# eladhoffer/convNet.pytorch

Hardware: NVIDIA H100
Metric: ResNet-50 images/sec (training step, synthetic 224x224) (higher is better)
Workload: dtype bf16

## Files before the change

convnet/pytorch_b200/csrc/conv3x3.cu:

```cuda
#include "common.cuh"
#include "host.h"
#include <stdlib.h>

namespace b200 {

constexpr int kHThreads = 384;
constexpr int kHTileM = 128;
constexpr int kHMaxA = 6, kHMaxB = 8;
constexpr int kHMaxTaps = 16;
constexpr int kHStatReplicas = 16;

struct HaloParams {
  int N, H, W, C, Kout;
  int RT, Wp;
  int tiles_per_img, m_tiles, n_tiles, block_n, c_chunks;
  int sa, sb;
  uint32_t a_bytes, a_box_bytes, b_bytes;
  int act;
  int has_res;
  double* stats;
  const float* bias;
  int ntaps, pad;
  int row_bytes;
  int b_stationary;
  int diag;
  uint16_t a_off[kHMaxTaps];
  uint16_t b_tap[kHMaxTaps];
};

template <int NTAPS, int KSTEPS, int BN>
__global__ void __launch_bounds__(kHThreads, 1)
conv_halo_kernel(const __grid_constant__ CUtensorMap tmX, const __grid_constant__ CUtensorMap tmB,
                 const __grid_constant__ CUtensorMap tmC, const __grid_constant__ CUtensorMap tmR,
                 const __grid_constant__ HaloParams p) {
  extern __shared__ uint8_t smem_raw[];
  __shared__ __align__(8) uint64_t a_full[kHMaxA], a_empty[kHMaxA], b_full[kHMaxB], b_empty[kHMaxB];
  __shared__ __align__(8) uint64_t res_bar, bstat_bar;

  const int warp = threadIdx.x >> 5, lane = threadIdx.x & 31;
  const uint32_t raw_addr = smem_u32(smem_raw);
  uint8_t* smem = smem_raw + (((raw_addr + 1023u) & ~1023u) - raw_addr);
  uint8_t* sA = smem;
  uint8_t* sB = sA + p.sa * p.a_bytes;
  const int b_slots = p.b_stationary ? p.c_chunks * p.ntaps : p.sb;
  uint8_t* epi = sB + b_slots * p.b_bytes;

  if (threadIdx.x == 0) {
    for (int i = 0; i < p.sa; ++i) { mbar_init(&a_full[i], 1); mbar_init(&a_empty[i], 8); }
    for (int i = 0; i < kHMaxB; ++i) { mbar_init(&b_full[i], 1); mbar_init(&b_empty[i], 8); }
    mbar_init(&bstat_bar, 1);
    mbar_init(&res_bar, 1);
    fence_mbar_init();
    prefetch_tmap(&tmX); prefetch_tmap(&tmB); prefetch_tmap(&tmC);
    if (p.has_res) prefetch_tmap(&tmR);
  }
  __syncthreads();
  const int t_start = p.diag ? static_cast<int>(blockIdx.x) / p.n_tiles : static_cast<int>(blockIdx.x);
  const int t_step = p.diag ? static_cast<int>(gridDim.x) / p.n_tiles : static_cast<int>(gridDim.x);
  const int total_tiles = p.diag ? p.m_tiles : p.m_tiles * p.n_tiles;
  const int own_n = static_cast<int>(blockIdx.x) % p.n_tiles;

  if (warp >= 8) {
    producer_setmaxnreg();
    if (warp == 8 && lane == 0) {
      int ia = 0, ib = 0; uint32_t pa = 0, pb = 0;
      const int cw = p.row_bytes >> 1;
      if (p.b_stationary && t_start < total_tiles) {
        mbar_arrive_expect_tx(&bstat_bar, static_cast<uint32_t>(p.c_chunks * NTAPS) * p.b_bytes);
        for (int cc = 0; cc < p.c_chunks; ++cc)
          for (int t = 0; t < NTAPS; ++t)
            tma_load_3d(&tmB, &bstat_bar, sB + (cc * NTAPS + t) * p.b_bytes, cc * cw, p.b_tap[t],
                        p.diag ? own_n * p.block_n : 0);
      }
      for (int tile = t_start; tile < total_tiles; tile += t_step) {
        const int m_tile = p.diag ? tile : tile / p.n_tiles, n_tile = p.diag ? own_n : tile - m_tile * p.n_tiles;
        const int img = m_tile / p.tiles_per_img;
        const int h0 = (m_tile - img * p.tiles_per_img) * p.RT;
        for (int cc = 0; cc < p.c_chunks; ++cc) {
          mbar_wait(&a_empty[ia], pa ^ 1u);
          mbar_arrive_expect_tx(&a_full[ia], p.a_box_bytes);
          tma_load_4d(&tmX, &a_full[ia], sA + ia * p.a_bytes, (p.diag ? n_tile : cc) * cw, -p.pad, h0 - p.pad, img);
          if (++ia == p.sa) { ia = 0; pa ^= 1u; }
          if (p.b_stationary) continue;
          for (int t = 0; t < NTAPS; ++t) {
            mbar_wait(&b_empty[ib], pb ^ 1u);
            mbar_arrive_expect_tx(&b_full[ib], p.b_bytes);
            tma_load_3d(&tmB, &b_full[ib], sB + ib * p.b_bytes, cc * cw, p.b_tap[t], n_tile * p.block_n);
            if (++ib == p.sb) { ib = 0; pb ^= 1u; }
          }
        }
      }
    }
    return;
  }
  consumer_setmaxnreg();

  const int wg = warp >> 2;
  const int r_lo = wg * 64 + (warp & 3) * 16 + (lane >> 2);
  const int c_lo = 2 * (lane & 3);
  const bool leader = threadIdx.x == 0;
  const uint64_t proto = make_smem_desc(0, 16, 8u * p.row_bytes, layout_type_for_row_bytes(p.row_bytes));
  const uint32_t a_wg = (64u * wg * p.row_bytes) >> 4;
  const int nbox = BN >> 6;
  const uint32_t box_bytes = static_cast<uint32_t>(p.RT * p.W) * 128u;
  const uint32_t box_pitch = (box_bytes + 1023u) & ~1023u;
  int srow[2];
  bool in_tile[2];
#pragma unroll
  for (int h = 0; h < 2; ++h) {
    const int v = r_lo + 8 * h;
    const int ry = v / p.Wp, cx = v - ry * p.Wp;
    srow[h] = ry * p.W + cx;
    in_tile[h] = (ry < p.RT) && (cx < p.W);
  }
  const int st_col = threadIdx.x % BN;
  const int st_rows = kHTileM / (256 / BN);
  const int st_row0 = (threadIdx.x / BN) * st_rows;
  int st_ntile = -1;
  float st_s1 = 0.f, st_s2 = 0.f;
  if (p.b_stationary && t_start < total_tiles) mbar_wait(&bstat_bar, 0);

  float acc[BN / 2];
  int ia = 0, ib = 0; uint32_t pa = 0, pb = 0;
  int local = 0;
  for (int tile = t_start; tile < total_tiles; tile += t_step, ++local) {
    const int m_tile = p.diag ? tile : tile / p.n_tiles, n_tile = p.diag ? own_n : tile - m_tile * p.n_tiles;
    const int img = m_tile / p.tiles_per_img;
    const int h0 = (m_tile - img * p.tiles_per_img) * p.RT;
    const int nbase = n_tile * BN;
    if (leader && local > 0) bulk_wait_group_read0();
    named_bar_sync(1, 256);
    if (leader && p.has_res) {
      fence_proxy_async();
      mbar_arrive_expect_tx(&res_bar, static_cast<uint32_t>(nbox) * box_bytes);
      for (int b = 0; b < nbox; ++b) tma_load_4d(&tmR, &res_bar, epi + b * box_pitch, nbase + b * 64, 0, h0, img);
    }

    wgmma_fence_acc(acc);
    int rel_a = -1, rel_b = -1;
    for (int cc = 0; cc < p.c_chunks; ++cc) {
      mbar_wait(&a_full[ia], pa);
      const uint64_t da0 = proto + (smem_u32(sA + ia * p.a_bytes) >> 4) + a_wg;
#pragma unroll
      for (int t = 0; t < NTAPS; ++t) {
        uint64_t db0;
        if (p.b_stationary) {
          db0 = proto + (smem_u32(sB + (cc * NTAPS + t) * p.b_bytes) >> 4);
        } else {
          mbar_wait(&b_full[ib], pb);
          db0 = proto + (smem_u32(sB + ib * p.b_bytes) >> 4);
        }
        const uint32_t tap_inc = (static_cast<uint32_t>(p.a_off[t]) * p.row_bytes) >> 4;
        wgmma_fence();
#pragma unroll
        for (int k = 0; k < KSTEPS; ++k)
          wgmma_bf16<0, 0>(acc, da0 + tap_inc + 2 * k, db0 + 2 * k, (cc | t | k) != 0 ? 1u : 0u);
        if (!p.b_stationary || t == NTAPS - 1) {
          wgmma_commit();
          wgmma_wait<1>();
          if (rel_b >= 0) release_stage(&b_empty[rel_b], lane);
          if (rel_a >= 0) release_stage(&a_empty[rel_a], lane);
          rel_a = (t == NTAPS - 1) ? ia : -1;
          rel_b = p.b_stationary ? -1 : ib;
        }
        if (!p.b_stationary && ++ib == p.sb) { ib = 0; pb ^= 1u; }
      }
      if (++ia == p.sa) { ia = 0; pa ^= 1u; }
    }
    wgmma_wait<0>();
    wgmma_fence_acc(acc);
    if (rel_b >= 0) release_stage(&b_empty[rel_b], lane);
    if (rel_a >= 0) release_stage(&a_empty[rel_a], lane);

    if (p.has_res) mbar_wait(&res_bar, static_cast<uint32_t>(local & 1));
#pragma unroll
    for (int h = 0; h < 2; ++h) {
      if (!in_tile[h] || h0 + (r_lo + 8 * h) / p.Wp >= p.H) continue;
      const int row = srow[h];
#pragma unroll
      for (int j = 0; j < BN / 2; j += 4) {
        const int c = 2 * j + c_lo;
        {
          uint32_t* dst = reinterpret_cast<uint32_t*>(epi + (c >> 6) * box_pitch + row * 128 +
                                                      ((((c & 63) >> 3) ^ (row & 7)) << 4) + (c & 7) * 2);
          float v0 = acc[j + 2 * h], v1 = acc[j + 2 * h + 1];
          if (p.bias != nullptr) { v0 += __ldg(p.bias + nbase + c); v1 += __ldg(p.bias + nbase + c + 1); }
          if (p.has_res) {
            const float2 t2 = unpack_bf16x2(*dst);
            v0 += t2.x;
            v1 += t2.y;
          }
          *dst = pack_bf16x2(apply_act(v0, p.act), apply_act(v1, p.act));
        }
      }
    }
    fence_proxy_async();
    named_bar_sync(1, 256);
    if (leader) {
      for (int b = 0; b < nbox; ++b) tma_store_4d(&tmC, epi + b * box_pitch, nbase + b * 64, 0, h0, img);
      bulk_commit_group();
    }
    if (p.stats != nullptr) {
      if (st_ntile != n_tile) {
        if (st_ntile >= 0) {
          double* dst = p.stats + (blockIdx.x % kHStatReplicas) * 2 * p.Kout + st_ntile * BN + st_col;
          atomicAdd(dst, (double)st_s1);
          atomicAdd(dst + p.Kout, (double)st_s2);
        }
        st_ntile = n_tile; st_s1 = 0.f; st_s2 = 0.f;
      }
      const int vrows = min(p.RT, p.H - h0) * p.W;
      const uint8_t* col = epi + (st_col >> 6) * box_pitch + (st_col & 7) * 2;
      const int j = (st_col & 63) >> 3;
      const int r_end = min(st_row0 + st_rows, vrows);
      for (int r = st_row0; r < r_end; ++r) {
        const float x = __bfloat162float(*reinterpret_cast<const __nv_bfloat16*>(col + r * 128 + ((j ^ (r & 7)) << 4)));
        st_s1 += x;
        st_s2 = fmaf(x, x, st_s2);
      }
    }
  }
  if (p.stats != nullptr && st_ntile >= 0) {
    double* dst = p.stats + (blockIdx.x % kHStatReplicas) * 2 * p.Kout + st_ntile * BN + st_col;
    atomicAdd(dst, (double)st_s1);
    atomicAdd(dst + p.Kout, (double)st_s2);
  }
  if (leader) bulk_wait_group0();
}

typedef void (*HaloKernelFn)(const __grid_constant__ CUtensorMap, const __grid_constant__ CUtensorMap,
                             const __grid_constant__ CUtensorMap, const __grid_constant__ CUtensorMap,
                             const __grid_constant__ HaloParams);
static HaloKernelFn halo_kernel_for(int ntaps, int block_n) {
  if (ntaps == 9)
    return block_n == 64 ? conv_halo_kernel<9, 4, 64> : block_n == 128 ? conv_halo_kernel<9, 4, 128>
         : block_n == 256 ? conv_halo_kernel<9, 4, 256> : nullptr;
  if (ntaps == 16)
    return block_n == 64 ? conv_halo_kernel<16, 1, 64> : block_n == 128 ? conv_halo_kernel<16, 1, 128>
         : block_n == 256 ? conv_halo_kernel<16, 1, 256> : nullptr;
  return nullptr;
}

static int enc4(CUtensorMap* tm, const void* base, int C, int W, int H, int N, int b0, int b1, int b2) {
  EncodeTiledFn fn = encode_tiled_fn();
  B200_REQUIRE(fn != nullptr, B200_ERR_CUDA, "cuTensorMapEncodeTiled entry point unavailable");
  cuuint64_t dims[4] = {(cuuint64_t)C, (cuuint64_t)W, (cuuint64_t)H, (cuuint64_t)N};
  cuuint64_t strides[3] = {(cuuint64_t)C * 2, (cuuint64_t)W * C * 2, (cuuint64_t)H * W * C * 2};
  cuuint32_t box[4] = {(cuuint32_t)b0, (cuuint32_t)b1, (cuuint32_t)b2, 1};
  cuuint32_t es[4] = {1, 1, 1, 1};
  CUresult r = fn(tm, CU_TENSOR_MAP_DATA_TYPE_BFLOAT16, 4, const_cast<void*>(base), dims, strides, box, es,
                  CU_TENSOR_MAP_INTERLEAVE_NONE, swizzle_for_row_bytes(b0 * 2), CU_TENSOR_MAP_L2_PROMOTION_L2_128B,
                  CU_TENSOR_MAP_FLOAT_OOB_FILL_NONE);
  B200_REQUIRE(r == CUDA_SUCCESS, B200_ERR_CUDA, "cuTensorMapEncodeTiled(4d) failed (%d) dims=(%d,%d,%d,%d) box=(%d,%d,%d)",
               (int)r, C, W, H, N, b0, b1, b2);
  return B200_OK;
}

bool halo_geometry_ok(int H, int W, int Cs, int R, int S, int pad) {
  const bool k3 = (R == 3 && S == 3 && pad == 1 && Cs % 64 == 0);
  const bool k4 = (R == 4 && S == 4 && pad == 0 && Cs == 16);
  if (!k3 && !k4) return false;
  const int Wp = W + S - 1;
  if (Wp > 128 || W < 8) return false;
  int RT = 128 / Wp;
  if (RT > H) RT = H;
  const int tiles = (H + RT - 1) / RT;
  return (double)H * W / (128.0 * tiles) >= 0.6;
}

bool halo_eligible(int H, int W, int Cs, int Nout, int R, int S, int pad) {
  if (!halo_geometry_ok(H, W, Cs, R, S, pad) || Nout % 64 != 0) return false;
  const int n_tiles = (Nout + 255) / 256;
  const int block_n = Nout / n_tiles;
  return Nout % n_tiles == 0 && block_n % 64 == 0 && 256 % block_n == 0;
}

int launch_halo(const void* src, const void* wmat, void* out, const void* res, const float* bias, int N, int H, int W,
                int Cs, int Nout, int R, int S, int pad, int dir, int act, double* stats, cudaStream_t stream, int window) {
  HaloParams p;
  memset(&p, 0, sizeof(p));
  p.diag = window > 0 ? 1 : 0;
  if (p.diag)
    B200_REQUIRE(window == 64 && Cs == Nout && Cs % 64 == 0 && R == 3 && S == 3, B200_ERR_UNSUPPORTED,
                 "conv halo: window mode needs window == 64, C == K, C %% 64 == 0 and a 3x3 filter (C=%d K=%d)", Cs, Nout);
  p.N = N; p.H = H; p.W = W; p.C = Cs; p.Kout = Nout;
  p.ntaps = R * S; p.pad = pad;
  p.row_bytes = (Cs == 16) ? 32 : 128;
  const int cw = p.row_bytes / 2;
  p.Wp = W + S - 1;
  p.RT = 128 / p.Wp;
  if (p.RT > H) p.RT = H;
  p.tiles_per_img = (H + p.RT - 1) / p.RT;
  p.m_tiles = N * p.tiles_per_img;
  p.n_tiles = p.diag ? Nout / 64 : (Nout + 255) / 256;
  p.block_n = Nout / p.n_tiles;
  p.c_chunks = p.diag ? 1 : Cs / cw;
  p.a_box_bytes = (uint32_t)(p.RT + R - 1) * p.Wp * p.row_bytes;
  uint32_t a_need = (uint32_t)(kHTileM + (R - 1) * p.Wp + (S - 1)) * p.row_bytes;
  if (a_need < p.a_box_bytes) a_need = p.a_box_bytes;
  p.a_bytes = (a_need + 1023u) & ~1023u;
  p.b_bytes = (uint32_t)p.block_n * p.row_bytes;
  p.act = act;
  p.has_res = res != nullptr;
  p.stats = stats;
  p.bias = bias;
  for (int r = 0; r < R; ++r)
    for (int s = 0; s < S; ++s) {
      const int t = r * S + s;
      p.b_tap[t] = (uint16_t)t;
      p.a_off[t] = (uint16_t)(dir == 0 ? r * p.Wp + s : (R - 1 - r) * p.Wp + (S - 1 - s));
    }
  const uint32_t box_pitch = (((uint32_t)(p.RT * W) * 128u) + 1023u) & ~1023u;
  const uint32_t epi_bytes = (uint32_t)(p.block_n / 64) * box_pitch;
  int budget = 212 * 1024 - (int)epi_bytes;
  const int b_all = p.c_chunks * p.ntaps * (int)p.b_bytes;
  p.b_stationary = ((p.n_tiles == 1 || p.diag) && b_all <= 80 * 1024) ? 1 : 0;
  B200_REQUIRE(!p.diag || p.b_stationary, B200_ERR_UNSUPPORTED, "conv halo: window mode expects resident weights");
  int b_region;
  if (p.b_stationary) {
    b_region = b_all;
    p.sb = 0;
    p.sa = (budget - b_region) / (int)p.a_bytes;
    if (p.sa > kHMaxA) p.sa = kHMaxA;
  } else {
    p.sa = 2;
    p.sb = (budget - p.sa * (int)p.a_bytes) / (int)p.b_bytes;
    if (p.sb > kHMaxB) p.sb = kHMaxB;
    if (p.sb >= 6 && (int)(3 * p.a_bytes + 4 * p.b_bytes) <= budget) {
      p.sa = 3;
      p.sb = (budget - 3 * (int)p.a_bytes) / (int)p.b_bytes;
      if (p.sb > kHMaxB) p.sb = kHMaxB;
    }
    b_region = p.sb * (int)p.b_bytes;
  }
  B200_REQUIRE(p.sa >= 2 && (p.b_stationary || p.sb >= 2), B200_ERR_UNSUPPORTED,
               "conv halo: shared memory budget exceeded (W=%d, block_n=%d)", W, p.block_n);
  CUtensorMap tmX, tmB, tmC, tmR;
  memset(&tmR, 0, sizeof(tmR));
  int rc = enc4(&tmX, src, Cs, W + S - 1 - 2 * pad, H + R - 1 - 2 * pad, N, cw, p.Wp, p.RT + R - 1);
  if (rc) return rc;
  {
    EncodeTiledFn fn = encode_tiled_fn();
    const int wc = p.diag ? window : Cs;
    cuuint64_t dims[3] = {(cuuint64_t)wc, (cuuint64_t)p.ntaps, (cuuint64_t)Nout};
    cuuint64_t strides[2] = {(cuuint64_t)wc * 2, (cuuint64_t)wc * p.ntaps * 2};
    cuuint32_t box[3] = {(cuuint32_t)cw, 1, (cuuint32_t)p.block_n};
    cuuint32_t es[3] = {1, 1, 1};
    CUresult r = fn(&tmB, CU_TENSOR_MAP_DATA_TYPE_BFLOAT16, 3, const_cast<void*>(wmat), dims, strides, box, es,
                    CU_TENSOR_MAP_INTERLEAVE_NONE, swizzle_for_row_bytes(p.row_bytes),
                    CU_TENSOR_MAP_L2_PROMOTION_L2_128B, CU_TENSOR_MAP_FLOAT_OOB_FILL_NONE);
    B200_REQUIRE(r == CUDA_SUCCESS, B200_ERR_CUDA, "conv halo: weight tensor map failed (%d)", (int)r);
  }
  rc = enc4(&tmC, out, Nout, W, H, N, 64, W, p.RT);
  if (rc) return rc;
  if (res) {
    rc = enc4(&tmR, res, Nout, W, H, N, 64, W, p.RT);
    if (rc) return rc;
  }
  const int smem_bytes = p.sa * (int)p.a_bytes + b_region + (int)epi_bytes + 1024;
  HaloKernelFn kfn = halo_kernel_for(p.ntaps, p.block_n);
  B200_REQUIRE(kfn != nullptr, B200_ERR_UNSUPPORTED, "conv halo: %d taps with block_n %d unsupported", p.ntaps, p.block_n);
  cudaError_t e = cudaFuncSetAttribute((const void*)kfn, cudaFuncAttributeMaxDynamicSharedMemorySize, smem_bytes);
  B200_REQUIRE(e == cudaSuccess, B200_ERR_CUDA, "conv halo: smem attribute (%d bytes): %s", smem_bytes, cudaGetErrorString(e));
  const int total = p.m_tiles * p.n_tiles;
  int grid = total < sm_count() ? total : sm_count();
  if (p.diag) {
    int per_n = sm_count() / p.n_tiles;
    if (per_n > p.m_tiles) per_n = p.m_tiles;
    if (per_n < 1) per_n = 1;
    grid = per_n * p.n_tiles;
  }
  if (getenv("B200_HALO_DEBUG"))
    fprintf(stderr, "[halo] dir=%d N=%d H=%d W=%d C=%d K=%d taps=%d block_n=%d n_tiles=%d m_tiles=%d bstat=%d diag=%d "
            "sa=%d sb=%d bias=%d res=%d act=%d stats=%d grid=%d\n", dir, N, H, W, Cs, Nout, p.ntaps, p.block_n,
            p.n_tiles, p.m_tiles, p.b_stationary, p.diag, p.sa, p.sb, bias != nullptr, res != nullptr, act,
            stats != nullptr, grid);
  b200::launch(kfn, grid, kHThreads, smem_bytes, stream, tmX, tmB, tmC, tmR, p);
  B200_CHECK_LAUNCH("conv_halo_kernel");
  return B200_OK;
}


constexpr int kWThreads = 384;
constexpr int kWMaxStages = 4;

struct HaloWgradParams {
  int N, H, W, K_out, C;
  int RT, Wp, tiles_per_img, m_tiles;
  int ntaps, pad, halo_rows;
  int x_row_bytes, cw, ncols;
  int c_chunks, k_tiles, units, splits, tiles_per_split;
  int stages;
  int window;
  uint32_t a_box_bytes, a_bytes, x_box_bytes, x_bytes;
  float* partial;
  uint16_t x_off[kHMaxTaps];
};

template <int R, int S>
__global__ void __launch_bounds__(kWThreads, 1)
conv_halo_wgrad_kernel(const __grid_constant__ CUtensorMap tmDy, const __grid_constant__ CUtensorMap tmX,
                       const __grid_constant__ HaloWgradParams p) {
  constexpr int kCols = S * 16;
  extern __shared__ uint8_t smem_raw[];
  __shared__ __align__(8) uint64_t full_bar[kWMaxStages], empty_bar[kWMaxStages];
  const int warp = threadIdx.x >> 5, lane = threadIdx.x & 31;
  const uint32_t raw_addr = smem_u32(smem_raw);
  uint8_t* smem = smem_raw + (((raw_addr + 1023u) & ~1023u) - raw_addr);
  const uint32_t stage_bytes = p.a_bytes + p.x_bytes;

  {
    uint4* z = reinterpret_cast<uint4*>(smem);
    const int n16 = static_cast<int>(p.stages * stage_bytes) >> 4;
    for (int i = threadIdx.x; i < n16; i += kWThreads) z[i] = make_uint4(0u, 0u, 0u, 0u);
  }
  if (threadIdx.x == 0) {
    for (int s = 0; s < p.stages; ++s) { mbar_init(&full_bar[s], 1); mbar_init(&empty_bar[s], 8); }
    fence_mbar_init();
    prefetch_tmap(&tmDy);
    prefetch_tmap(&tmX);
  }
  fence_proxy_async();
  __syncthreads();

  const int split = blockIdx.x / p.units;
  const int unit = blockIdx.x - split * p.units;
  const int k_tile = unit % p.k_tiles;
  const int cc = unit / p.k_tiles;
  const int k0 = k_tile * kHTileM;
  const int t_begin = split * p.tiles_per_split;
  const int t_end = min(p.m_tiles, t_begin + p.tiles_per_split);
  const int ntiles = t_end - t_begin;
  const int nA = min(2, (p.K_out - k0 + 63) / 64);
  if (ntiles <= 0) return;

  if (warp >= 8) {
    producer_setmaxnreg();
    if (warp == 8 && lane == 0) {
      int stage = 0; uint32_t phase = 0;
      const uint32_t tx = nA * p.a_box_bytes + p.x_box_bytes;
      for (int tile = t_begin; tile < t_end; ++tile) {
        const int img = tile / p.tiles_per_img;
        const int h0 = (tile - img * p.tiles_per_img) * p.RT;
        mbar_wait(&empty_bar[stage], phase ^ 1u);
        uint8_t* sa = smem + stage * stage_bytes;
        mbar_arrive_expect_tx(&full_bar[stage], tx);
        for (int j = 0; j < nA; ++j) tma_load_4d(&tmDy, &full_bar[stage], sa + j * 16384, k0 + j * 64, 0, h0, img);
        tma_load_4d(&tmX, &full_bar[stage], sa + p.a_bytes, cc * p.cw + (p.window ? k0 : 0), -p.pad, h0 - p.pad, img);
        if (++stage == p.stages) { stage = 0; phase ^= 1u; }
      }
    }
    return;
  }
  consumer_setmaxnreg();

  const int wg = warp >> 2;
  const bool wg_on = wg < nA;
  const uint64_t protoA = make_smem_desc(0, 16384, 1024, 1);
  const uint64_t protoX = make_smem_desc(0, p.x_row_bytes, 8u * p.x_row_bytes, layout_type_for_row_bytes(p.x_row_bytes));
  uint32_t row_inc[R];
#pragma unroll
  for (int r = 0; r < R; ++r) row_inc[r] = (static_cast<uint32_t>(p.x_off[r * S]) * p.x_row_bytes) >> 4;
  const uint32_t kx_inc = (16u * p.x_row_bytes) >> 4;
  float acc[R][kCols / 2];
#pragma unroll
  for (int r = 0; r < R; ++r) wgmma_fence_acc(acc[r]);
  int stage = 0, prev = 0; uint32_t phase = 0;
  for (int i = 0; i < ntiles; ++i) {
    mbar_wait(&full_bar[stage], phase);
    if (wg_on) {
      const uint32_t a_addr = smem_u32(smem + stage * stage_bytes);
      const uint64_t da0 = protoA + ((a_addr + wg * 16384) >> 4);
      const uint64_t dx0 = protoX + ((a_addr + p.a_bytes) >> 4);
      wgmma_fence();
#pragma unroll
      for (int k = 0; k < 8; ++k) {
        const uint32_t scale = (k != 0 || i != 0) ? 1u : 0u;
#pragma unroll
        for (int r = 0; r < R; ++r)
          wgmma_bf16<1, 1>(acc[r], da0 + k * 128, dx0 + row_inc[r] + k * kx_inc, scale);
      }
      wgmma_commit();
      wgmma_wait<1>();
    }
    if (i > 0) release_stage(&empty_bar[prev], lane);
    prev = stage;
    if (++stage == p.stages) { stage = 0; phase ^= 1u; }
  }
  wgmma_wait<0>();
#pragma unroll
  for (int r = 0; r < R; ++r) wgmma_fence_acc(acc[r]);
  release_stage(&empty_bar[prev], lane);
  if (!wg_on) return;

  const int row = wg * 64 + (warp & 3) * 16 + (lane >> 2);
  const int c_lo = 2 * (lane & 3);
#pragma unroll
  for (int h = 0; h < 2; ++h) {
    float* dst = p.partial + ((static_cast<long long>(unit) * p.splits + split) * kHTileM + row + 8 * h) * p.ncols;
#pragma unroll
    for (int r = 0; r < R; ++r)
#pragma unroll
      for (int j = 0; j < kCols / 2; j += 4)
        *reinterpret_cast<float2*>(dst + r * kCols + 2 * j + c_lo) = make_float2(acc[r][j + 2 * h], acc[r][j + 2 * h + 1]);
  }
}

__global__ void __launch_bounds__(256) conv_halo_wgrad_reduce_kernel(const float* __restrict__ partial,
                                                                     float* __restrict__ dw, int K_out, int ntaps, int C,
                                                                     int cw, int k_tiles, int splits, int ncols) {
  __shared__ float4 red[8][32];
  const int c4n = C >> 2;
  const long long total = static_cast<long long>(K_out) * ntaps * c4n;
  const int lane = threadIdx.x & 31, w = threadIdx.x >> 5, nw = blockDim.x >> 5;
  for (long long base = static_cast<long long>(blockIdx.x) * 32; base < total; base += static_cast<long long>(gridDim.x) * 32) {
    const long long idx = base + lane;
    float4 acc = make_float4(0.f, 0.f, 0.f, 0.f);
    int c = 0, tap = 0, k = 0;
    if (idx < total) {
      c = static_cast<int>(idx % c4n) * 4;
      tap = static_cast<int>((idx / c4n) % ntaps);
      k = static_cast<int>(idx / (static_cast<long long>(c4n) * ntaps));
      const int k_tile = k >> 7, row = k & 127;
      const int cc = c / cw;
      const int unit = cc * k_tiles + k_tile;
      const float* src = partial + ((static_cast<long long>(unit) * splits) * kHTileM + row) * ncols + tap * cw + (c - cc * cw);
      for (int s2 = w; s2 < splits; s2 += nw) {
        const float4 v = __ldcg(reinterpret_cast<const float4*>(src + static_cast<long long>(s2) * kHTileM * ncols));
        acc.x += v.x; acc.y += v.y; acc.z += v.z; acc.w += v.w;
      }
    }
    red[w][lane] = acc;
    __syncthreads();
    if (w == 0 && idx < total) {
      for (int j = 1; j < nw; ++j) {
        const float4 v = red[j][lane];
        acc.x += v.x; acc.y += v.y; acc.z += v.z; acc.w += v.w;
      }
      float4* d = reinterpret_cast<float4*>(dw + (static_cast<long long>(k) * ntaps + tap) * C + c);
      float4 o = *d;
      o.x += acc.x; o.y += acc.y; o.z += acc.z; o.w += acc.w;
      *d = o;
    }
    __syncthreads();
  }
}

bool halo_wgrad_eligible(int H, int W, int C, int K_out, int R, int S, int pad) {
  if (!halo_geometry_ok(H, W, C, R, S, pad)) return false;
  return K_out % 64 == 0;
}

int launch_halo_wgrad(const void* x, const void* dy, float* dw, void* workspace, size_t workspace_bytes, int N, int H,
                      int W, int C, int K_out, int R, int S, int pad, cudaStream_t stream, int window) {
  HaloWgradParams p;
  memset(&p, 0, sizeof(p));
  p.window = window;
  if (window)
    B200_REQUIRE(window == 128 && C == K_out && C % 128 == 0, B200_ERR_UNSUPPORTED,
                 "conv halo wgrad: window mode needs window == 128 and C == K, C %% 128 == 0 (C=%d K=%d)", C, K_out);
  p.N = N; p.H = H; p.W = W; p.K_out = K_out; p.C = C;
  p.ntaps = R * S; p.pad = pad;
  p.cw = 16;
  p.x_row_bytes = p.cw * 2;
  p.ncols = p.ntaps * p.cw;
  p.Wp = W + S - 1;
  p.RT = 128 / p.Wp;
  if (p.RT > H) p.RT = H;
  p.halo_rows = p.RT + R - 1;
  p.tiles_per_img = (H + p.RT - 1) / p.RT;
  p.m_tiles = N * p.tiles_per_img;
  p.c_chunks = (window ? window : C) / p.cw;
  p.k_tiles = (K_out + kHTileM - 1) / kHTileM;
  p.units = p.c_chunks * p.k_tiles;
  int splits = sm_count() / p.units;
  if (splits < 1) splits = 1;
  if (splits > p.m_tiles) splits = p.m_tiles;
  p.tiles_per_split = (p.m_tiles + splits - 1) / splits;
  p.splits = (p.m_tiles + p.tiles_per_split - 1) / p.tiles_per_split;
  p.a_box_bytes = (uint32_t)(p.RT * p.Wp) * 128u;
  p.a_bytes = 2 * 16384;
  p.x_box_bytes = (uint32_t)(p.halo_rows * p.Wp) * p.x_row_bytes;
  int max_off = 0;
  for (int r = 0; r < R; ++r)
    for (int s = 0; s < S; ++s) {
      p.x_off[r * S + s] = (uint16_t)(r * p.Wp + s);
      if (r * p.Wp + s > max_off) max_off = r * p.Wp + s;
    }
  uint32_t x_need = (uint32_t)(kHTileM + max_off) * p.x_row_bytes;
  if (x_need < p.x_box_bytes) x_need = p.x_box_bytes;
  p.x_bytes = (x_need + 1023u) & ~1023u;
  p.stages = (212 * 1024) / (int)(p.a_bytes + p.x_bytes);
  if (p.stages > kWMaxStages) p.stages = kWMaxStages;
  B200_REQUIRE(p.stages >= 2, B200_ERR_UNSUPPORTED, "conv halo wgrad: shared memory budget exceeded (W=%d)", W);
  const size_t need = (size_t)p.units * p.splits * kHTileM * p.ncols * sizeof(float);
  B200_REQUIRE(workspace != nullptr && workspace_bytes >= need, B200_ERR_INVALID,
               "conv halo wgrad: workspace of %zu bytes needed (%zu given)", need, workspace_bytes);
  p.partial = reinterpret_cast<float*>(workspace);
  CUtensorMap tmDy, tmX;
  int rc = enc4(&tmDy, dy, K_out, W, H, N, 64, p.Wp, p.RT);
  if (rc) return rc;
  rc = enc4(&tmX, x, C, W + S - 1 - 2 * pad, H + R - 1 - 2 * pad, N, p.cw, p.Wp, p.halo_rows);
  if (rc) return rc;
  const int smem_bytes = p.stages * (int)(p.a_bytes + p.x_bytes) + 1024;
  const void* kfn = (p.ntaps == 9) ? (const void*)conv_halo_wgrad_kernel<3, 3> : (const void*)conv_halo_wgrad_kernel<4, 4>;
  cudaError_t e = cudaFuncSetAttribute(kfn, cudaFuncAttributeMaxDynamicSharedMemorySize, smem_bytes);
  B200_REQUIRE(e == cudaSuccess, B200_ERR_CUDA, "conv halo wgrad: smem attribute (%d bytes): %s", smem_bytes,
               cudaGetErrorString(e));
  if (getenv("B200_HALO_DEBUG"))
    fprintf(stderr, "[halo_wgrad] N=%d H=%d W=%d C=%d K=%d taps=%d k_tiles=%d c_chunks=%d m_tiles=%d units=%d "
            "splits=%d tiles_per_split=%d stages=%d grid=%d\n", N, H, W, C, K_out, p.ntaps, p.k_tiles, p.c_chunks,
            p.m_tiles, p.units, p.splits, p.tiles_per_split, p.stages, p.units * p.splits);
  if (p.ntaps == 9)
    b200::launch(conv_halo_wgrad_kernel<3, 3>, p.units * p.splits, kWThreads, smem_bytes, stream, tmDy, tmX, p);
  else
    b200::launch(conv_halo_wgrad_kernel<4, 4>, p.units * p.splits, kWThreads, smem_bytes, stream, tmDy, tmX, p);
  B200_CHECK_LAUNCH("conv_halo_wgrad_kernel");
  const int Cw = window ? window : C;
  const long long total = (long long)K_out * p.ntaps * (Cw / 4);
  long long blocks64 = (total + 31) / 32;
  if (blocks64 > 16LL * sm_count()) blocks64 = 16LL * sm_count();
  const int blocks = (int)blocks64;
  b200::launch(conv_halo_wgrad_reduce_kernel, blocks, 32 * wgrad_reduce_warps(p.splits), 0, stream, p.partial, dw, K_out, p.ntaps, Cw, p.cw, p.k_tiles, p.splits,
                                                            p.ncols);
  B200_CHECK_LAUNCH("conv_halo_wgrad_reduce_kernel");
  return B200_OK;
}

}
```

Measured before the change: 6694.

## Double M tile height for block_n=64 halo conv to improve B reuse

Adds an MH template parameter so each consumer warpgroup issues two stacked 64-row wgmma per k-step, giving a 256-row M tile when block_n is 64. The host picks MH=2 if it gives more image rows per tile and still fits shared memory, and otherwise falls back to MH=1. The aim is to reuse each weight tile across twice as many output rows and cut per-tile overheads. The cost is doubled accumulator registers, a larger A buffer that may leave fewer pipeline stages, and fewer tiles, which can hurt SM load balance.

Result: faster. 6801 (median of 6 runs) (+1.6%).

```diff
diff --git a/convnet/pytorch_b200/csrc/conv3x3.cu b/convnet/pytorch_b200/csrc/conv3x3.cu
--- a/convnet/pytorch_b200/csrc/conv3x3.cu
+++ b/convnet/pytorch_b200/csrc/conv3x3.cu
@@ -28,7 +28,7 @@
   uint16_t b_tap[kHMaxTaps];
 };
 
-template <int NTAPS, int KSTEPS, int BN>
+template <int NTAPS, int KSTEPS, int BN, int MH>
 __global__ void __launch_bounds__(kHThreads, 1)
 conv_halo_kernel(const __grid_constant__ CUtensorMap tmX, const __grid_constant__ CUtensorMap tmB,
                  const __grid_constant__ CUtensorMap tmC, const __grid_constant__ CUtensorMap tmR,
@@ -96,31 +96,33 @@
   consumer_setmaxnreg();
 
   const int wg = warp >> 2;
-  const int r_lo = wg * 64 + (warp & 3) * 16 + (lane >> 2);
+  const int r_lo = wg * 64 * MH + (warp & 3) * 16 + (lane >> 2);
   const int c_lo = 2 * (lane & 3);
   const bool leader = threadIdx.x == 0;
   const uint64_t proto = make_smem_desc(0, 16, 8u * p.row_bytes, layout_type_for_row_bytes(p.row_bytes));
-  const uint32_t a_wg = (64u * wg * p.row_bytes) >> 4;
+  const uint32_t a_wg = (64u * MH * wg * p.row_bytes) >> 4;
+  const uint32_t a_half = (64u * p.row_bytes) >> 4;
   const int nbox = BN >> 6;
   const uint32_t box_bytes = static_cast<uint32_t>(p.RT * p.W) * 128u;
   const uint32_t box_pitch = (box_bytes + 1023u) & ~1023u;
-  int srow[2];
-  bool in_tile[2];
-#pragma unroll
-  for (int h = 0; h < 2; ++h) {
-    const int v = r_lo + 8 * h;
-    const int ry = v / p.Wp, cx = v - ry * p.Wp;
-    srow[h] = ry * p.W + cx;
-    in_tile[h] = (ry < p.RT) && (cx < p.W);
+  int srow[2 * MH], ry[2 * MH];
+  bool in_tile[2 * MH];
+#pragma unroll
+  for (int q = 0; q < 2 * MH; ++q) {
+    const int v = r_lo + 64 * (q >> 1) + 8 * (q & 1);
+    ry[q] = v / p.Wp;
+    const int cx = v - ry[q] * p.Wp;
+    srow[q] = ry[q] * p.W + cx;
+    in_tile[q] = (ry[q] < p.RT) && (cx < p.W);
   }
   const int st_col = threadIdx.x % BN;
-  const int st_rows = kHTileM / (256 / BN);
+  const int st_rows = kHTileM * MH / (256 / BN);
   const int st_row0 = (threadIdx.x / BN) * st_rows;
   int st_ntile = -1;
   float st_s1 = 0.f, st_s2 = 0.f;
   if (p.b_stationary && t_start < total_tiles) mbar_wait(&bstat_bar, 0);
 
-  float acc[BN / 2];
+  float acc[MH][BN / 2];
   int ia = 0, ib = 0; uint32_t pa = 0, pb = 0;
   int local = 0;
   for (int tile = t_start; tile < total_tiles; tile += t_step, ++local) {
@@ -136,7 +138,8 @@
       for (int b = 0; b < nbox; ++b) tma_load_4d(&tmR, &res_bar, epi + b * box_pitch, nbase + b * 64, 0, h0, img);
     }
 
-    wgmma_fence_acc(acc);
+#pragma unroll
+    for (int mh = 0; mh < MH; ++mh) wgmma_fence_acc(acc[mh]);
     int rel_a = -1, rel_b = -1;
     for (int cc = 0; cc < p.c_chunks; ++cc) {
       mbar_wait(&a_full[ia], pa);
@@ -154,7 +157,9 @@
         wgmma_fence();
 #pragma unroll
         for (int k = 0; k < KSTEPS; ++k)
-          wgmma_bf16<0, 0>(acc, da0 + tap_inc + 2 * k, db0 + 2 * k, (cc | t | k) != 0 ? 1u : 0u);
+#pragma unroll
+          for (int mh = 0; mh < MH; ++mh)
+            wgmma_bf16<0, 0>(acc[mh], da0 + tap_inc + mh * a_half + 2 * k, db0 + 2 * k, (cc | t | k) != 0 ? 1u : 0u);
         if (!p.b_stationary || t == NTAPS - 1) {
           wgmma_commit();
           wgmma_wait<1>();
@@ -168,22 +173,23 @@
       if (++ia == p.sa) { ia = 0; pa ^= 1u; }
     }
     wgmma_wait<0>();
-    wgmma_fence_acc(acc);
+#pragma unroll
+    for (int mh = 0; mh < MH; ++mh) wgmma_fence_acc(acc[mh]);
     if (rel_b >= 0) release_stage(&b_empty[rel_b], lane);
     if (rel_a >= 0) release_stage(&a_empty[rel_a], lane);
 
     if (p.has_res) mbar_wait(&res_bar, static_cast<uint32_t>(local & 1));
 #pragma unroll
-    for (int h = 0; h < 2; ++h) {
-      if (!in_tile[h] || h0 + (r_lo + 8 * h) / p.Wp >= p.H) continue;
-      const int row = srow[h];
+    for (int q = 0; q < 2 * MH; ++q) {
+      if (!in_tile[q] || h0 + ry[q] >= p.H) continue;
+      const int row = srow[q];
 #pragma unroll
       for (int j = 0; j < BN / 2; j += 4) {
         const int c = 2 * j + c_lo;
         {
           uint32_t* dst = reinterpret_cast<uint32_t*>(epi + (c >> 6) * box_pitch + row * 128 +
                                                       ((((c & 63) >> 3) ^ (row & 7)) << 4) + (c & 7) * 2);
-          float v0 = acc[j + 2 * h], v1 = acc[j + 2 * h + 1];
+          float v0 = acc[q >> 1][j + 2 * (q & 1)], v1 = acc[q >> 1][j + 2 * (q & 1) + 1];
           if (p.bias != nullptr) { v0 += __ldg(p.bias + nbase + c); v1 += __ldg(p.bias + nbase + c + 1); }
           if (p.has_res) {
             const float2 t2 = unpack_bf16x2(*dst);
@@ -231,13 +237,13 @@
 typedef void (*HaloKernelFn)(const __grid_constant__ CUtensorMap, const __grid_constant__ CUtensorMap,
                              const __grid_constant__ CUtensorMap, const __grid_constant__ CUtensorMap,
                              const __grid_constant__ HaloParams);
-static HaloKernelFn halo_kernel_for(int ntaps, int block_n) {
+static HaloKernelFn halo_kernel_for(int ntaps, int block_n, int mh) {
   if (ntaps == 9)
-    return block_n == 64 ? conv_halo_kernel<9, 4, 64> : block_n == 128 ? conv_halo_kernel<9, 4, 128>
-         : block_n == 256 ? conv_halo_kernel<9, 4, 256> : nullptr;
+    return block_n == 64 ? (mh == 2 ? conv_halo_kernel<9, 4, 64, 2> : conv_halo_kernel<9, 4, 64, 1>)
+         : block_n == 128 ? conv_halo_kernel<9, 4, 128, 1> : block_n == 256 ? conv_halo_kernel<9, 4, 256, 1> : nullptr;
   if (ntaps == 16)
-    return block_n == 64 ? conv_halo_kernel<16, 1, 64> : block_n == 128 ? conv_halo_kernel<16, 1, 128>
-         : block_n == 256 ? conv_halo_kernel<16, 1, 256> : nullptr;
+    return block_n == 64 ? (mh == 2 ? conv_halo_kernel<16, 1, 64, 2> : conv_halo_kernel<16, 1, 64, 1>)
+         : block_n == 128 ? conv_halo_kernel<16, 1, 128, 1> : block_n == 256 ? conv_halo_kernel<16, 1, 256, 1> : nullptr;
   return nullptr;
 }
 
@@ -288,17 +294,9 @@
   p.row_bytes = (Cs == 16) ? 32 : 128;
   const int cw = p.row_bytes / 2;
   p.Wp = W + S - 1;
-  p.RT = 128 / p.Wp;
-  if (p.RT > H) p.RT = H;
-  p.tiles_per_img = (H + p.RT - 1) / p.RT;
-  p.m_tiles = N * p.tiles_per_img;
   p.n_tiles = p.diag ? Nout / 64 : (Nout + 255) / 256;
   p.block_n = Nout / p.n_tiles;
   p.c_chunks = p.diag ? 1 : Cs / cw;
-  p.a_box_bytes = (uint32_t)(p.RT + R - 1) * p.Wp * p.row_bytes;
-  uint32_t a_need = (uint32_t)(kHTileM + (R - 1) * p.Wp + (S - 1)) * p.row_bytes;
-  if (a_need < p.a_box_bytes) a_need = p.a_box_bytes;
-  p.a_bytes = (a_need + 1023u) & ~1023u;
   p.b_bytes = (uint32_t)p.block_n * p.row_bytes;
   p.act = act;
   p.has_res = res != nullptr;
@@ -310,31 +308,43 @@
       p.b_tap[t] = (uint16_t)t;
       p.a_off[t] = (uint16_t)(dir == 0 ? r * p.Wp + s : (R - 1 - r) * p.Wp + (S - 1 - s));
     }
-  const uint32_t box_pitch = (((uint32_t)(p.RT * W) * 128u) + 1023u) & ~1023u;
-  const uint32_t epi_bytes = (uint32_t)(p.block_n / 64) * box_pitch;
-  int budget = 212 * 1024 - (int)epi_bytes;
   const int b_all = p.c_chunks * p.ntaps * (int)p.b_bytes;
   p.b_stationary = ((p.n_tiles == 1 || p.diag) && b_all <= 80 * 1024) ? 1 : 0;
   B200_REQUIRE(!p.diag || p.b_stationary, B200_ERR_UNSUPPORTED, "conv halo: window mode expects resident weights");
-  int b_region;
-  if (p.b_stationary) {
-    b_region = b_all;
-    p.sb = 0;
-    p.sa = (budget - b_region) / (int)p.a_bytes;
-    if (p.sa > kHMaxA) p.sa = kHMaxA;
-  } else {
-    p.sa = 2;
-    p.sb = (budget - p.sa * (int)p.a_bytes) / (int)p.b_bytes;
-    if (p.sb > kHMaxB) p.sb = kHMaxB;
-    if (p.sb >= 6 && (int)(3 * p.a_bytes + 4 * p.b_bytes) <= budget) {
-      p.sa = 3;
-      p.sb = (budget - 3 * (int)p.a_bytes) / (int)p.b_bytes;
+  int mh = 0, b_region = 0;
+  uint32_t epi_bytes = 0;
+  for (int cand = p.block_n == 64 ? 2 : 1; cand >= 1 && mh == 0; --cand) {
+    p.RT = min(kHTileM * cand / p.Wp, H);
+    if (cand == 2 && p.RT <= min(kHTileM / p.Wp, H)) continue;
+    p.a_box_bytes = (uint32_t)(p.RT + R - 1) * p.Wp * p.row_bytes;
+    uint32_t a_need = (uint32_t)(kHTileM * cand + (R - 1) * p.Wp + (S - 1)) * p.row_bytes;
+    if (a_need < p.a_box_bytes) a_need = p.a_box_bytes;
+    p.a_bytes = (a_need + 1023u) & ~1023u;
+    const uint32_t box_pitch = (((uint32_t)(p.RT * W) * 128u) + 1023u) & ~1023u;
+    epi_bytes = (uint32_t)(p.block_n / 64) * box_pitch;
+    const int budget = 212 * 1024 - (int)epi_bytes;
+    if (p.b_stationary) {
+      b_region = b_all;
+      p.sb = 0;
+      p.sa = (budget - b_region) / (int)p.a_bytes;
+      if (p.sa > kHMaxA) p.sa = kHMaxA;
+    } else {
+      p.sa = 2;
+      p.sb = (budget - p.sa * (int)p.a_bytes) / (int)p.b_bytes;
       if (p.sb > kHMaxB) p.sb = kHMaxB;
-    }
-    b_region = p.sb * (int)p.b_bytes;
-  }
-  B200_REQUIRE(p.sa >= 2 && (p.b_stationary || p.sb >= 2), B200_ERR_UNSUPPORTED,
+      if (p.sb >= 6 && (int)(3 * p.a_bytes + 4 * p.b_bytes) <= budget) {
+        p.sa = 3;
+        p.sb = (budget - 3 * (int)p.a_bytes) / (int)p.b_bytes;
+        if (p.sb > kHMaxB) p.sb = kHMaxB;
+      }
+      b_region = p.sb * (int)p.b_bytes;
+    }
+    if (p.sa >= 2 && (p.b_stationary || p.sb >= 2)) mh = cand;
+  }
+  B200_REQUIRE(mh > 0, B200_ERR_UNSUPPORTED,
                "conv halo: shared memory budget exceeded (W=%d, block_n=%d)", W, p.block_n);
+  p.tiles_per_img = (H + p.RT - 1) / p.RT;
+  p.m_tiles = N * p.tiles_per_img;
   CUtensorMap tmX, tmB, tmC, tmR;
   memset(&tmR, 0, sizeof(tmR));
   int rc = enc4(&tmX, src, Cs, W + S - 1 - 2 * pad, H + R - 1 - 2 * pad, N, cw, p.Wp, p.RT + R - 1);
@@ -358,7 +368,7 @@
     if (rc) return rc;
   }
   const int smem_bytes = p.sa * (int)p.a_bytes + b_region + (int)epi_bytes + 1024;
-  HaloKernelFn kfn = halo_kernel_for(p.ntaps, p.block_n);
+  HaloKernelFn kfn = halo_kernel_for(p.ntaps, p.block_n, mh);
   B200_REQUIRE(kfn != nullptr, B200_ERR_UNSUPPORTED, "conv halo: %d taps with block_n %d unsupported", p.ntaps, p.block_n);
   cudaError_t e = cudaFuncSetAttribute((const void*)kfn, cudaFuncAttributeMaxDynamicSharedMemorySize, smem_bytes);
   B200_REQUIRE(e == cudaSuccess, B200_ERR_CUDA, "conv halo: smem attribute (%d bytes): %s", smem_bytes, cudaGetErrorString(e));
@@ -370,11 +380,13 @@
     if (per_n < 1) per_n = 1;
     grid = per_n * p.n_tiles;
   }
-  if (getenv("B200_HALO_DEBUG"))
+  if (getenv("B200_HALO_DEBUG")) {
+    const int max_tiles = p.diag ? (p.m_tiles + grid / p.n_tiles - 1) / (grid / p.n_tiles) : (total + grid - 1) / grid;
     fprintf(stderr, "[halo] dir=%d N=%d H=%d W=%d C=%d K=%d taps=%d block_n=%d n_tiles=%d m_tiles=%d bstat=%d diag=%d "
-            "sa=%d sb=%d bias=%d res=%d act=%d stats=%d grid=%d\n", dir, N, H, W, Cs, Nout, p.ntaps, p.block_n,
-            p.n_tiles, p.m_tiles, p.b_stationary, p.diag, p.sa, p.sb, bias != nullptr, res != nullptr, act,
-            stats != nullptr, grid);
+            "sa=%d sb=%d bias=%d res=%d act=%d stats=%d grid=%d max_tiles=%d c_chunks=%d RT=%d tile_m=%d\n", dir, N, H,
+            W, Cs, Nout, p.ntaps, p.block_n, p.n_tiles, p.m_tiles, p.b_stationary, p.diag, p.sa, p.sb, bias != nullptr,
+            res != nullptr, act, stats != nullptr, grid, max_tiles, p.c_chunks, p.RT, kHTileM * mh);
+  }
   b200::launch(kfn, grid, kHThreads, smem_bytes, stream, tmX, tmB, tmC, tmR, p);
   B200_CHECK_LAUNCH("conv_halo_kernel");
   return B200_OK;
```
